# mic-rud/RABBIT-Transcoding

Measured on AMD Instinct MI355X. Metric: transcoded point-cloud frames/sec, R5->R3, higher is better.
Workload: dtype u16/i32

## Files before the change

### rabbit-transcoding_amd/csrc/rbt_encode.h

```cpp
#pragma once
#include "rbt_cabac.h"
#include "rbt_recon.h"
#include "rbt_filter.h"

RBT_CONST uint16_t k_lambda16[76] = {3,    3,    4,    4,    5,    5,    6,    7,    8,    9,    10,   11,   12,   14,   15,   17,   19,   22,   24,
                                     27,   30,   34,   38,   43,   48,   54,   61,   68,   77,   86,   97,   108,  122,  137,  153,  172,  193,  217,
                                     244,  273,  307,  344,  387,  434,  487,  547,  614,  689,  773,  868,  974,  1093, 1227, 1378, 1546, 1736, 1948,
                                     2187, 2454, 2755, 3092, 3471, 3896, 4373, 4909, 5510, 6185, 6942, 7792, 8747, 9818, 11020, 12370, 13884, 15585, 17493};
RBT_CONST uint8_t k_intra_cand[11] = {0, 1, 26, 10, 2, 6, 14, 18, 22, 30, 34};
#define RBT_SPLIT_BITS 48
#define RBT_PARTIAL_COST 0x0FFFFFFF
#define RBT_AN_GOOD 2
#define RBT_AN_SKIPPED 0x0FFFFFFE

struct RbtEncLds {
  RbtReconLds rc;
  int16_t lvl[32 * 32];
};
struct RbtEntropyLds {
  uint8_t scan[3][4][64];
  uint8_t cu_l2[81], cu_md[81], cu_fl[81];
  alignas(16) int16_t lv[64 * 64 * 3 / 2];
};
#define RBT_ENTROPY_LDS_BYTES(tl2) (sizeof(RbtEntropyLds) - sizeof(int16_t) * (64 * 64 * 3 / 2 - (3 << (2 * (tl2) - 1))))
RBT_DEV RBT_LDS_AS int16_t* en_lv(RBT_LDS_AS RbtEntropyLds* l, int c, int log2_ctb) { const int nn = 1 << (2 * log2_ctb); return l->lv + (c == 0 ? 0 : c == 1 ? nn : nn + (nn >> 2)); }

RBT_DEV int en_wave_sum(int v, RBT_LDS_AS RbtEncLds* l) { (void)l; return rbt_wave_sum(v); }
#ifdef RBT_HOSTEMU
static inline int en_had8x8_sum_host(const int* r) {
  int t[64], sum = 0;
  for (int y = 0; y < 8; y++) for (int k = 0; k < 8; k++) { int s = 0; for (int x = 0; x < 8; x++) s += (__builtin_popcount(k & x) & 1) ? -r[y * 8 + x] : r[y * 8 + x]; t[y * 8 + k] = s; }
  for (int k = 0; k < 8; k++) for (int x = 0; x < 8; x++) { int s = 0; for (int y = 0; y < 8; y++) s += (__builtin_popcount(k & y) & 1) ? -t[y * 8 + x] : t[y * 8 + x]; sum += s < 0 ? -s : s; }
  return sum;
}
#define EN_HAD8X8_ACC(vr, acc) (acc) += en_had8x8_sum_host(vr)
#else
RBT_DEV int en_had_stage(int v, int partner, int upper) { return upper ? partner - v : partner + v; }
RBT_DEV int en_had8x8_abs(int v) {
  const int lane = (int)threadIdx.x & 63;
  v = en_had_stage(v, __builtin_amdgcn_update_dpp(0, v, 0x141, 0xF, 0xF, false), lane & 4);
  v = en_had_stage(v, __builtin_amdgcn_update_dpp(0, v, 0xB1, 0xF, 0xF, false), lane & 1);
  v = en_had_stage(v, __builtin_amdgcn_update_dpp(0, v, 0x4E, 0xF, 0xF, false), lane & 2);
  v = en_had_stage(v, __builtin_amdgcn_update_dpp(0, v, 0x128, 0xF, 0xF, false), lane & 8);
  v = en_had_stage(v, __builtin_amdgcn_ds_swizzle(v, 0x401F), lane & 16);
  v = en_had_stage(v, __builtin_amdgcn_ds_bpermute((lane ^ 32) << 2, v), lane & 32);
  return v < 0 ? -v : v;
}
#define EN_HAD8X8_ACC(vr, acc) (acc) += en_had8x8_abs(vr)
#endif
RBT_DEV int en_occ_unit(const RbtFrame* f, int ux, int uy) { return ux < f->occ4_w && uy < f->occ4_h && f->occ4[(size_t)uy * f->occ4_w + ux] != 0; }
RBT_DEV int en_round_mean(int sum, int cnt) { return sum >= 0 ? (sum + cnt / 2) / cnt : -((-sum + cnt / 2) / cnt); }
RBT_DEV int en_occ_unit_value(const uint16_t* occ, int ow, int oh, int s, int w4, int h4, int i, int j) {
  const int x_lo = (4 * rbt_max(i - 1, 0)) / s, x_hi = rbt_min(ow - 1, (4 * rbt_min(i + 1, w4 - 1) + 3) / s), y_lo = (4 * rbt_max(j - 1, 0)) / s, y_hi = rbt_min(oh - 1, (4 * rbt_min(j + 1, h4 - 1) + 3) / s);
  int any = 0;
  for (int y = y_lo; y <= y_hi; y++) for (int x = x_lo; x <= x_hi; x++) any |= occ[(size_t)y * ow + x] != 0;
  return any;
}
RBT_DEV int en_rq_offset(int lf_is0, int lf_is1, int xy_sum) { return lf_is0 ? (xy_sum <= 2 ? 180 : 145) : (lf_is1 ? 195 : 230); }
RBT_DEV int en_chroma_qp(const RbtFrame* f, const RbtSlice* sl, int c_idx, int qp_y) {
  int off = c_idx == 1 ? f->cfg.cb_qp_offset + sl->cb_qp_offset : f->cfg.cr_qp_offset + sl->cr_qp_offset;
  int bdo = 6 * (f->cfg.bit_depth - 8);
  int qpi = rbt_clip3(-bdo, 57, qp_y + off);
  return (qpi < 0 ? qpi : rbt_chroma_qp(qpi)) + bdo;
}

struct EnCtbNb { int cx, cy, ctb, w, h, left, above_left, above, above_right; };
RBT_DEV int en_avail(const EnCtbNb* q, int xc, int yc, int xn, int yn) {
  if (xn < 0 || yn < 0 || xn >= q->w || yn >= q->h) return 0;
  const int dx = xn - q->cx, dy = yn - q->cy;
  if (dy >= q->ctb) return 0;
  if (dy < 0) return dx < 0 ? q->above_left : (dx < q->ctb ? q->above : q->above_right);
  if (dx < 0) return q->left;
  if (dx >= q->ctb) return 0;
  return rc_z_before(dx >> 2, dy >> 2, (xc - q->cx) >> 2, (yc - q->cy) >> 2);
}
struct RbtAnalyseLds {
  int32_t nb[132], nbf[132], ref[100];
  uint16_t src[65 * 66];
  int32_t cost[3][16]; uint8_t mode[3][16], split[3][16];
  uint8_t hint[64];
};
RBT_DEV int en_nb_unit_av(const EnCtbNb* q, int p, int x0, int y0, int S) { int xn, yn; rc_nb_unit_xy(p, x0, y0, S, 0, &xn, &yn); return en_avail(q, x0, y0, xn, yn); }
RBT_DEV void en_analyse_ctb(RbtFrame* f, const RbtSlice* slices, int ctb_addr, RBT_LDS_AS RbtAnalyseLds* l) {
  const RbtStreamCfg gcopy = rc_cfg_uni(&f->cfg); const RbtStreamCfg* g = &gcopy;
  int ctb = 1 << g->log2_ctb, rx = ctb_addr % g->w_ctb, ry = ctb_addr / g->w_ctb, cx = rx << g->log2_ctb, cy = ry << g->log2_ctb;
  const int my_slice = f->ctb_slice[ctb_addr];
  const RbtSlice* sl = &slices[my_slice];
  RBT_LDS_AS RbtAnalyseLds* rl = l;
  EnCtbNb nbq; nbq.cx = cx; nbq.cy = cy; nbq.ctb = ctb; nbq.w = g->w; nbq.h = g->h;
  nbq.left = rx > 0 && f->ctb_slice[ctb_addr - 1] == my_slice;
  nbq.above = ry > 0 && f->ctb_slice[ctb_addr - g->w_ctb] == my_slice;
  nbq.above_left = rx > 0 && ry > 0 && f->ctb_slice[ctb_addr - g->w_ctb - 1] == my_slice;
  nbq.above_right = ry > 0 && rx + 1 < g->w_ctb && f->ctb_slice[ctb_addr - g->w_ctb + 1] == my_slice;
  const uint16_t* srcp = f->src[0];
  const int hints = f->hint_dm != nullptr, hint_w4 = f->hint_w4, hint_h4 = f->hint_h4, satd_on = f->enc_tools & RBT_ET_SATD;
  int nq = ctb > 32 ? 2 : 1, qs = ctb > 32 ? 32 : ctb;
  for (int q = 0; q < nq * nq; q++) {
    int qx = cx + (q % nq) * 32, qy = cy + (q / nq) * 32;
    if (nq > 1 && (qx >= g->w || qy >= g->h)) continue;
    if (!(RBT_ABLATE & 0x100))
#pragma unroll 4
    RBT_PAR_FOR(i, 65 * 16) {
      const int x4 = i & 15, yy = (i >> 4) - 1, x = qx + 4 * x4, y = qy + yy;
      RbtU2 v; v.x = 0; v.y = 0;
      if (y >= 0 && y < g->h && x < g->w) v = *(const RbtU2*)(srcp + (size_t)y * g->w + x);
      RBT_LDS_AS uint16_t* d = &l->src[(yy + 1) * 66 + 4 * x4 + 1];
      d[0] = (uint16_t)v.x; d[1] = (uint16_t)(v.x >> 16); d[2] = (uint16_t)v.y; d[3] = (uint16_t)(v.y >> 16);
    }
    RBT_PAR_FOR(i, 65) { const int x = qx - 1, y = qy + i - 1; l->src[i * 66] = (x >= 0 && y >= 0 && y < g->h) ? srcp[(size_t)y * g->w + x] : 0; }
    if (hints && !(RBT_ABLATE & 0x400)) RBT_PAR_FOR(u, 64) {
      const int hx = (qx >> 2) + (u & 7), hy = (qy >> 2) + (u >> 3); int v = 255;
      if (hx < hint_w4 && hy < hint_h4) { const size_t hk = (size_t)hy * hint_w4 + hx; if ((f->hint_pm[hk] & RBT_PM_MODE_MASK) == RBT_MODE_INTRA) v = f->hint_dm[hk] & 63; }
      l->hint[u] = (uint8_t)v;
    }
    RBT_SYNC_LDS();
    for (int si = 2; si >= 0; si--) {
      int S = 8 << si; if (S > qs) continue;
      int nb = qs / S, lg = 3 + si;
      for (int b = 0; b < nb * nb; b++) {
        int x0 = qx + (b % nb) * S, y0 = qy + (b / nb) * S, best = 0x7FFFFFFF, bmode = 0;
        if (x0 >= g->w || y0 >= g->h) best = 0;
        else if (x0 + S > g->w || y0 + S > g->h) best = RBT_PARTIAL_COST;
        else if (si < 2 && 2 * S <= qs && (RBT_UNI(l->cost[si + 1][((b / nb) >> 1) * (nb >> 1) + ((b % nb) >> 1)]) <= (f->lossless ? 0 : RBT_AN_GOOD) * 4 * S * S ||
                                            RBT_UNI(l->cost[si + 1][((b / nb) >> 1) * (nb >> 1) + ((b % nb) >> 1)]) == RBT_AN_SKIPPED)) best = RBT_AN_SKIPPED;
        else {
          const int tot = 4 * S + 1, bx0 = x0 - qx, by0 = y0 - qy;
          if (!(RBT_ABLATE & 0x200)) {
          uint64_t m; RBT_VBALLOT(m, p, rc_nb_units(S, 0), en_nb_unit_av(&nbq, p, x0, y0, S));
          RcNbMap nm; rc_nb_map(&nm, m, S, 0);
          RBT_PAR_FOR(i, tot) {
            int v = 1 << (g->bit_depth - 1);
            if (m) { const int j = rc_nb_source(&nm, i); v = j < 2 * S ? l->src[(by0 + 2 * S - j) * 66 + bx0] : l->src[by0 * 66 + bx0 + j - 2 * S]; }
            rl->nb[i] = v;
          }
          RBT_SYNC_LDS();
          rc_intra_filter_apply(g, lg, rl->nb, rl->nbf);
          }
          int parent = -1;
          if (si == 0 && qs >= 16) { const int pb = ((b / nb) >> 1) * (nb >> 1) + ((b % nb) >> 1); if (RBT_UNI(l->cost[1][pb]) < RBT_PARTIAL_COST) parent = RBT_UNI(l->mode[1][pb]); }
          uint64_t hc = 0; int nh = 0;
          if (hints) {
            int any = 0;
            hc = 1ull << 6; nh = 2;
            if (!(RBT_ABLATE & 0x400)) for (int q = 0; q < 4; q++) {
              const int v = RBT_UNI(l->hint[((by0 + (q >> 1) * (S >> 1)) >> 2) * 8 + ((bx0 + (q & 1) * (S >> 1)) >> 2)]);
              if (v < 35) {
                any = 1;
                int dup = 0; for (int t = 0; t < nh; t++) dup |= (int)((hc >> (6 * t)) & 63) == v;
                if (!dup) { hc |= (uint64_t)v << (6 * nh); nh++; }
              }
            }
            if (!any) { hc |= (26ull << 12) | (10ull << 18); nh = 4; }
          }
          int coarse = 0;
          RBT_VEC(int, v_last); RBT_VEC(int, v_keep);
          RBT_VFOR(p, 64) { RBT_V(v_last, p) = 0; RBT_V(v_keep, p) = 0; }
          for (int k = 0; k < 15; k++) {
            int mode;
            if (best == 0) break;
            if (hints) { if (k >= nh) break; mode = (int)((hc >> (6 * k)) & 63); }
            else if (parent >= 0) {
              if (k >= 9) break;
              if (k < 4) mode = k == 0 ? 0 : (k == 1 ? 1 : (k == 2 ? 26 : 10));
              else if (parent >= 2) { mode = parent + (k - 6); if (mode < 2 || mode > 34 || mode == 10 || mode == 26) continue; }
              else { if (k >= 7) break; mode = k == 4 ? 2 : (k == 5 ? 18 : 34); }
            } else if (k < 11) mode = k_intra_cand[k];
            else { if (k == 11) coarse = bmode; if (coarse < 2) break; mode = coarse + (k == 11 ? -2 : k == 12 ? -1 : k == 13 ? 1 : 2); if (mode < 2 || mode > 34) continue; }
            RBT_LDS_AS int32_t* fin = rc_intra_filter_needed(0, lg, mode) ? rl->nbf : rl->nb;
            RcIntraCtx qc; if (!(RBT_ABLATE & 0x800)) rc_intra_setup(g, 0, lg, mode, fin, rl->ref, &qc); else { qc.N = S; qc.log2 = lg; qc.mode = mode; qc.c_idx = 0; qc.maxv = 1023; qc.ang = 1; qc.ver = mode >= 18; qc.dc = 1; qc.edge = 0; }
            int part = (RBT_ABLATE & 0x1000) ? 1 + k : 0;
#define EN_BODY(PV) RBT_PAR_FOR(i, S * S) { const int x = i & (S - 1), y = i >> lg, r = (int)l->src[(by0 + y + 1) * 66 + bx0 + x + 1] - (PV); part += rbt_abs(r); RBT_V(v_last, i & 63) = r; }
            if (!(RBT_ABLATE & 0x1000)) RC_INTRA_KINDS(&qc, fin, rl->ref, EN_BODY);
#undef EN_BODY
            int sad = en_wave_sum(part, (RBT_LDS_AS RbtEncLds*)0);
            if (sad < best) { best = sad; bmode = mode; if (S == 8) { RBT_VFOR(p, 64) RBT_V(v_keep, p) = RBT_V(v_last, p); } }
            RBT_SYNC_LDS();
          }
          if (satd_on && best > 0 && S == 8 && !(RBT_ABLATE & (0x2000 | 0x1000))) {
            int acc = 0; EN_HAD8X8_ACC(v_keep, acc);
            best = (en_wave_sum(acc, (RBT_LDS_AS RbtEncLds*)0) + 4) >> 3;
          } else if (satd_on && best > 0 && !(RBT_ABLATE & 0x2000)) {
            RBT_LDS_AS int32_t* fin = rc_intra_filter_needed(0, lg, bmode) ? rl->nbf : rl->nb;
            RcIntraCtx qc; rc_intra_setup(g, 0, lg, bmode, fin, rl->ref, &qc);
            int acc = 0; const int tw = S >> 3;
#define EN_BODY(PV) for (int tix = 0; tix < tw * tw; tix++) { \
              const int tx = (tix % tw) * 8, ty = (tix / tw) * 8; \
              RBT_VEC(int, v_r); \
              RBT_VFOR(p, 64) { const int x = tx + (p & 7), y = ty + (p >> 3); RBT_V(v_r, p) = (int)l->src[(by0 + y + 1) * 66 + bx0 + x + 1] - (PV); } \
              EN_HAD8X8_ACC(v_r, acc); }
            RC_INTRA_KINDS(&qc, fin, rl->ref, EN_BODY);
#undef EN_BODY
            best = (en_wave_sum(acc, (RBT_LDS_AS RbtEncLds*)0) + 4) >> 3;
            RBT_SYNC_LDS();
          }
        }
    if (RBT_LANE0) { l->cost[si][b] = best; l->mode[si][b] = (uint8_t)bmode; }
      }
    }
    RBT_SYNC_LDS();
    int lam = k_lambda16[rbt_clip3(0, 75, sl->qp + 6 * (g->bit_depth - 8))], pen = (lam * RBT_SPLIT_BITS) >> 4;
    for (int si = 1; si < 3; si++) {
      int S = 8 << si; if (S > qs) break;
      int nb = qs / S, nbc = nb * 2;
      RBT_PAR_FOR(b, nb * nb) {
        int bx = b % nb, by = b / nb;
        int child = l->cost[si - 1][(2 * by) * nbc + 2 * bx] + l->cost[si - 1][(2 * by) * nbc + 2 * bx + 1] + l->cost[si - 1][(2 * by + 1) * nbc + 2 * bx] +
                    l->cost[si - 1][(2 * by + 1) * nbc + 2 * bx + 1] + pen;
        int split = child < l->cost[si][b];
        l->split[si][b] = (uint8_t)split;
        if (split) l->cost[si][b] = child;
      }
      RBT_SYNC_LDS();
    }
    int n8 = qs / 8;
    RBT_PAR_FOR(u, n8 * n8) {
      int ux = u % n8, uy = u / n8, x = qx + ux * 8, y = qy + uy * 8;
      if (x < g->w && y < g->h) {
        int lg = 3, mode = l->mode[0][uy * n8 + ux];
        int inside32 = qx + 32 <= g->w && qy + 32 <= g->h, inside16 = (x & ~15) + 16 <= g->w && (y & ~15) + 16 <= g->h;
        int b16 = (uy / 2) * (n8 / 2) + ux / 2;
        int split32 = qs >= 32 ? (inside32 ? l->split[2][0] : 1) : 1;
        int split16 = qs >= 16 ? (inside16 ? l->split[1][b16] : 1) : 1;
        if (qs >= 32 && !split32) { lg = 5; mode = l->mode[2][0]; }
        else if (qs >= 16 && !split16) { lg = 4; mode = l->mode[1][b16]; }
        int k = (y >> 3) * f->w8 + (x >> 3);
        f->cu_log2[k] = (uint8_t)lg; f->cu_mode[k] = (uint8_t)mode;
      }
    }
    RBT_SYNC_LDS();
  }
}

template <int LOG2> RBT_DEV void en_fwd_transform_n(int is_dst, int bd, RBT_LDS_AS RbtReconLdsCore* r) {
  constexpr int N = 1 << LOG2; const int s1 = LOG2 + bd - 9, s2 = LOG2 + 6;
  RBT_PAR_FOR(i, N * N) {
    int k = i & (N - 1), y = i >> LOG2, s = 0;
#pragma unroll
    for (int x = 0; x < N; x++) s += rc_tcoef(r, N, is_dst, k, x) * r->res[y * N + x];
    r->tmp[i] = (int16_t)(s1 > 0 ? (s + (1 << (s1 - 1))) >> s1 : s);
  }
  RBT_SYNC_LDS();
  RBT_PAR_FOR(i, N * N) {
    int kh = i & (N - 1), kv = i >> LOG2, s = 0;
#pragma unroll
    for (int y = 0; y < N; y++) s += rc_tcoef(r, N, is_dst, kv, y) * r->tmp[y * N + kh];
    r->res[i] = (int16_t)rbt_clip3(-32768, 32767, (s + (1 << (s2 - 1))) >> s2);
  }
  RBT_SYNC_LDS();
}
template <int LOG2> RBT_DEV void en_fwd_transform_pair_n(int bd, RBT_LDS_AS RbtReconLdsCore* r) {
  constexpr int N = 1 << LOG2, NN = N * N; const int s1 = LOG2 + bd - 9, s2 = LOG2 + 6;
  RBT_PAR_FOR(i, 2 * NN) {
    const int b = i >> (2 * LOG2), j = i & (NN - 1), k = j & (N - 1), y = j >> LOG2; int s = 0;
#pragma unroll
    for (int x = 0; x < N; x++) s += rc_tcoef(r, N, 0, k, x) * r->res[b * 256 + y * N + x];
    r->tmp[b * 256 + j] = (int16_t)(s1 > 0 ? (s + (1 << (s1 - 1))) >> s1 : s);
  }
  RBT_SYNC_LDS();
  RBT_PAR_FOR(i, 2 * NN) {
    const int b = i >> (2 * LOG2), j = i & (NN - 1), kh = j & (N - 1), kv = j >> LOG2; int s = 0;
#pragma unroll
    for (int y = 0; y < N; y++) s += rc_tcoef(r, N, 0, kv, y) * r->tmp[b * 256 + y * N + kh];
    r->res[b * 256 + j] = (int16_t)rbt_clip3(-32768, 32767, (s + (1 << (s2 - 1))) >> s2);
  }
  RBT_SYNC_LDS();
}
RBT_DEV void en_fwd_transform_32(int bd, RBT_LDS_AS RbtReconLdsCore* r) {
#ifdef RBT_HOSTEMU
  en_fwd_transform_n<5>(0, bd, r);
#else
  mf_mm32<false>(r->dct, 32, 1, r->res, r->tmp, 5 + bd - 9, 0);
  mf_mm32<true>(r->dct, 32, 1, r->tmp, r->res, 5 + 6, 1);
#endif
}
RBT_DEV void en_fwd_transform(int log2, int is_dst, int bd, RBT_LDS_AS RbtReconLdsCore* r) {
  if (log2 == 2) en_fwd_transform_n<2>(is_dst, bd, r);
  else if (log2 == 3) en_fwd_transform_n<3>(0, bd, r);
  else if (log2 == 4) en_fwd_transform_n<4>(0, bd, r);
  else en_fwd_transform_32(bd, r);
}
RBT_DEV int en_quant(int log2, int qp, int bd, int is_intra, RBT_LDS_AS RbtEncLds* l) {
  int N = 1 << log2, qbits = 14 + qp / 6 + (15 - bd - log2), sc = k_quant_scale[qp % 6], part = 0;
  long long add = (long long)(is_intra ? 171 : 85) << (qbits - 9);
  RBT_PAR_FOR(i, N * N) {
    int c = l->rc.res[i], a = rbt_abs(c);
    long long q = ((long long)a * sc + add) >> qbits;
    if (q > 32767) q = 32767;
    l->lvl[i] = (int16_t)(c < 0 ? -q : q);
    part += q != 0;
  }
  int nz = en_wave_sum(part, l);
  return nz;
}
RBT_DEV int en_code_tb(RbtFrame* f, int c_idx, int x0, int y0, int log2, int qp, int is_intra, RBT_LDS_AS RbtEncLds* l) {
  const RbtStreamCfg* g = &f->cfg;
  int N = 1 << log2, pw = c_idx ? g->cw : g->w, bd = g->bit_depth, maxv = (1 << bd) - 1;
  const uint16_t* sp = f->src[c_idx]; uint16_t* rp = f->pix[c_idx]; int16_t* cp = f->coef[c_idx];
  RBT_PAR_FOR(i, N * N) { int x = i & (N - 1), y = i >> log2; l->rc.res[i] = (int16_t)((int)sp[(size_t)(y0 + y) * pw + x0 + x] - (int)l->rc.pred[i]); }
  RBT_SYNC_LDS();
  int occ_none = 0;
  if (f->occ4 != nullptr) {
    const int sh = c_idx ? 1 : 0;
#define EN_TBP_OCC(i) en_occ_unit(f, ((x0 + ((i) & (N - 1))) << sh) >> 2, ((y0 + ((i) >> log2)) << sh) >> 2)
    int pc = 0, ps = 0;
    RBT_PAR_FOR(i, N * N) { if (EN_TBP_OCC(i)) { pc++; ps += l->rc.res[i]; } }
    const int cnt = en_wave_sum(pc, l);
    occ_none = cnt == 0;
    if (cnt > 0 && cnt < N * N) {
      const int mean = en_round_mean(en_wave_sum(ps, l), cnt);
      RBT_PAR_FOR(i, N * N) { if (!EN_TBP_OCC(i)) l->rc.res[i] = (int16_t)mean; }
      RBT_SYNC_LDS();
    }
#undef EN_TBP_OCC
  }
  int nz;
  if (occ_none) { RBT_PAR_FOR(i, N * N) l->lvl[i] = 0; nz = 0; }
  else if (f->lossless) {
    int part = 0;
    RBT_PAR_FOR(i, N * N) { l->lvl[i] = l->rc.res[i]; part += l->rc.res[i] != 0; }
    nz = en_wave_sum(part, l);
  } else {
    en_fwd_transform(log2, c_idx == 0 && log2 == 2 && is_intra, bd, &l->rc);
    nz = en_quant(log2, qp, bd, is_intra, l);
  }
  RBT_SYNC_LDS();
  if (nz) { RBT_PAR_FOR(i, N * N) { int x = i & (N - 1), y = i >> log2; cp[(size_t)(y0 + y) * pw + x0 + x] = l->lvl[i]; } }
  if (nz && !f->lossless) {
    int bd_shift = bd + log2 - 5, scale = (16 * k_dequant_scale[qp % 6]) << (qp / 6);
    long long add = 1ll << (bd_shift - 1);
    RBT_PAR_FOR(i, N * N) { long long v = ((long long)l->lvl[i] * scale + add) >> bd_shift; l->rc.res[i] = (int16_t)(v < -32768 ? -32768 : (v > 32767 ? 32767 : v)); }
// ... 1066 lines not shown
```

### rabbit-transcoding_amd/csrc/rbt_recon.h

```cpp
#pragma once
#include "rbt_tables.h"
#include "rbt_types.h"
#include "rbt_mfma.h"

struct RbtReconLdsCore {
  int32_t nb[132];
  alignas(16) int16_t res[32 * 32];
  alignas(16) int16_t tmp[32 * 32];
  int8_t dct[32 * 32]; int8_t dst[16];
};
struct RbtReconLds : RbtReconLdsCore {
  int32_t nbf[132];
  int32_t ref[100];
  int32_t ref2[100];
  uint16_t pred[32 * 32];
};
RBT_DEV void rc_stage_tables(RBT_LDS_AS RbtReconLdsCore* l) {
  RBT_PAR_FOR(i, 1024) l->dct[i] = k_dct32[i >> 5][i & 31];
  RBT_PAR_FOR(i, 16) l->dst[i] = k_dst4[i >> 2][i & 3];
  RBT_SYNC_LDS();
}

RBT_DEV int rc_morton(int x4, int y4) {
  int z = 0;
  for (int b = 0; b < 4; b++) z |= (((x4 >> b) & 1) << (2 * b)) | (((y4 >> b) & 1) << (2 * b + 1));
  return z;
}
RBT_DEV int rc_z_before(int ax, int ay, int bx, int by) {
  const int dx = ax ^ bx, dy = ay ^ by, x_decides = dy < dx && dy < (dx ^ dy);
  return x_decides ? ax < bx : ay < by;
}
RBT_DEV int rc_avail(const RbtFrame* f, int xc, int yc, int xn, int yn) {
  const RbtStreamCfg* g = &f->cfg;
  if (xn < 0 || yn < 0 || xn >= g->w || yn >= g->h) return 0;
  int L = g->log2_ctb, an = (yn >> L) * g->w_ctb + (xn >> L), ac = (yc >> L) * g->w_ctb + (xc >> L);
  if (an > ac || f->ctb_slice[an] != f->ctb_slice[ac]) return 0;
  if (an == ac) {
    int m = (1 << L) - 1;
    if (rc_morton((xn & m) >> 2, (yn & m) >> 2) >= rc_morton((xc & m) >> 2, (yc & m) >> 2)) return 0;
  }
  if (g->cip && (f->pm[(yn >> 2) * g->w4 + (xn >> 2)] & RBT_PM_MODE_MASK) != RBT_MODE_INTRA) return 0;
  return 1;
}
RBT_DEV int rc_tcoef(const RBT_LDS_AS RbtReconLdsCore* l, int N, int is_dst, int k, int n) { return is_dst ? l->dst[k * 4 + n] : l->dct[k * (32 / N) * 32 + n]; }

RBT_DEV int rc_intra_angle(int mode) {
  const int k = mode <= 18 ? mode - 2 : 34 - mode, d = k < 8 ? 8 - k : k - 8;
  const uint64_t M = 0ull | (2ull << 6) | (5ull << 12) | (9ull << 18) | (13ull << 24) | (17ull << 30) | (21ull << 36) | (26ull << 42) | (32ull << 48);
  const int a = (int)((M >> (6 * d)) & 63);
  return k <= 8 ? a : -a;
}
RBT_DEV int rc_intra_inv_angle(int mode) {
  const int d = mode < 18 ? 18 - mode : mode - 18;
  const uint64_t lo = 256ull | (315ull << 16) | (390ull << 32) | (482ull << 48), hi = 630ull | (910ull << 16) | (1638ull << 32) | (4096ull << 48);
  return -(int)(((d < 4 ? lo : hi) >> (16 * (d & 3))) & 0xFFFF);
}
RBT_DEV int rc_level_scale(int r) { return (int)((0x484039332D28ull >> (8 * r)) & 255); }
RBT_DEV int rbt_wave_sum(int v) {
#ifdef RBT_HOSTEMU
  return v;
#else
  int x = v;
  x += __builtin_amdgcn_update_dpp(0, x, 0xB1, 0xF, 0xF, false);
  x += __builtin_amdgcn_update_dpp(0, x, 0x4E, 0xF, 0xF, false);
  x += __builtin_amdgcn_update_dpp(0, x, 0x141, 0xF, 0xF, false);
  x += __builtin_amdgcn_update_dpp(0, x, 0x140, 0xF, 0xF, false);
  return __builtin_amdgcn_readlane(x, 0) + __builtin_amdgcn_readlane(x, 16) + __builtin_amdgcn_readlane(x, 32) + __builtin_amdgcn_readlane(x, 48);
#endif
}
struct RcNbMap { uint64_t m; int two_n, usl, nu, lo, hi, run; };
RBT_DEV int rc_nb_unit_of(const RcNbMap* q, int i) { return i < q->two_n ? i >> q->usl : (i == q->two_n ? q->nu : q->nu + 1 + ((i - q->two_n - 1) >> q->usl)); }
RBT_DEV int rc_nb_unit_lo(const RcNbMap* q, int u) { return u < q->nu ? u << q->usl : (u == q->nu ? q->two_n : q->two_n + 1 + ((u - q->nu - 1) << q->usl)); }
RBT_DEV int rc_nb_unit_hi(const RcNbMap* q, int u) { return u < q->nu ? (u << q->usl) + (1 << q->usl) - 1 : (u == q->nu ? q->two_n : q->two_n + ((u - q->nu) << q->usl)); }
RBT_DEV void rc_nb_unit_xy(int p, int x0, int y0, int N, int sh, int* xn, int* yn) {
  const int usl = 2 - sh, nu = (2 * N) >> usl;
  if (p < nu) { *xn = x0 - 1; *yn = y0 + 2 * N - 1 - (p << usl); }
  else if (p == nu) { *xn = x0 - 1; *yn = y0 - 1; }
  else { *xn = x0 + ((p - nu - 1) << usl); *yn = y0 - 1; }
}
RBT_DEV int rc_nb_units(int N, int sh) { return ((4 * N) >> (2 - sh)) + 1; }
RBT_DEV void rc_nb_map(RcNbMap* q, uint64_t m, int N, int sh) {
  q->m = m; q->two_n = 2 * N; q->usl = 2 - sh; q->nu = (2 * N) >> q->usl; q->lo = q->hi = -1; q->run = 0;
  if (m) {
    const int ua = __builtin_ctzll(m), ub = 63 - __builtin_clzll(m); const uint64_t t = m >> ua;
    q->lo = rc_nb_unit_lo(q, ua); q->hi = rc_nb_unit_hi(q, ub); q->run = (t & (t + 1)) == 0;
  }
}
RBT_DEV int rc_nb_source(const RcNbMap* q, int i) {
  if (q->run) return rbt_clip3(q->lo, q->hi, i);
  const int u = rc_nb_unit_of(q, i); const uint64_t t = q->m & ((2ull << u) - 1);
  if (!t) return q->lo;
  const int uj = 63 - __builtin_clzll(t);
  return uj == u ? i : rc_nb_unit_hi(q, uj);
}
RBT_DEV int rc_intra_filter_needed(int c_idx, int log2, int mode) {
  const int N = 1 << log2;
  if (c_idx != 0 || mode == 1 || N == 4) return 0;
  const int md = rbt_min(rbt_abs(mode - 26), rbt_abs(mode - 10)), thr = N == 8 ? 7 : (N == 16 ? 1 : 0);
  return md > thr;
}
RBT_DEV void rc_intra_filter_apply(const RbtStreamCfg* g, int log2, RBT_LDS_AS int32_t* nb, RBT_LDS_AS int32_t* alt) {
  const int N = 1 << log2, bd = g->bit_depth, tot = 4 * N + 1;
  int corner = nb[2 * N], bl = nb[0], tr = nb[4 * N];
  int strong = g->strong_intra && N == 32 && rbt_abs(corner + tr - 2 * nb[2 * N + 32]) < (1 << (bd - 5)) &&
               rbt_abs(corner + bl - 2 * nb[2 * N - 32]) < (1 << (bd - 5));
  RBT_PAR_FOR(i, tot) {
    int v;
    if (i == 0 || i == 4 * N) v = nb[i];
    else if (strong) {
      if (i == 2 * N) v = corner;
      else if (i < 2 * N) { int k = 2 * N - 1 - i; v = ((63 - k) * corner + (k + 1) * bl + 32) >> 6; }
      else { int k = i - 2 * N - 1; v = ((63 - k) * corner + (k + 1) * tr + 32) >> 6; }
    } else v = (nb[i - 1] + 2 * nb[i] + nb[i + 1] + 2) >> 2;
    alt[i] = v;
  }
  RBT_SYNC_LDS();
}
RBT_DEV RBT_LDS_AS int32_t* rc_intra_filter(const RbtStreamCfg* g, int c_idx, int log2, int mode, RBT_LDS_AS int32_t* nb, RBT_LDS_AS int32_t* alt) {
  if (!rc_intra_filter_needed(c_idx, log2, mode)) return nb;
  if (!(RBT_ABLATE & 4)) rc_intra_filter_apply(g, log2, nb, alt);
  return alt;
}
struct RcIntraCtx { int N, log2, mode, c_idx, maxv, ang, ver, dc, edge; };
RBT_DEV void rc_intra_setup(const RbtStreamCfg* g, int c_idx, int log2, int mode, RBT_LDS_AS int32_t* nb, RBT_LDS_AS int32_t* ref, RcIntraCtx* q) {
  const int N = 1 << log2, bd = g->bit_depth;
  q->N = N; q->log2 = log2; q->mode = mode; q->c_idx = c_idx; q->maxv = (1 << bd) - 1; q->ang = 0; q->ver = mode >= 18; q->dc = 0; q->edge = 0;
#define RC_LEFT(y) nb[2 * N - 1 - (y)]
#define RC_TOP(x) nb[2 * N + 1 + (x)]
  if (mode == 1) {
    int part = 0;
    if (!(RBT_ABLATE & 8)) RBT_PAR_FOR(p, 2 * N) part += p < N ? RC_TOP(p) : RC_LEFT(p - N);
    q->dc = (N + rbt_wave_sum(part)) >> (log2 + 1); q->edge = c_idx == 0 && N < 32;
  } else if (mode >= 2) {
    const int ang = rc_intra_angle(mode), ver = mode >= 18, last = (N * ang) >> 5;
    const int inv = (mode >= 11 && mode <= 25) ? rc_intra_inv_angle(mode) : 0;
    q->ang = ang; q->edge = c_idx == 0 && N < 32 && (mode == 26 || mode == 10);
    if (!(RBT_ABLATE & 8)) RBT_PAR_FOR(i, 3 * N + 1) {
      int x = i - N, v = 0;
      if (x >= 0 && x <= N) v = ver ? RC_TOP(x - 1) : RC_LEFT(x - 1);
      else if (x < 0) { if (ang < 0 && last < -1 && x >= last) { int k = -1 + ((x * inv + 128) >> 8); v = ver ? RC_LEFT(k) : RC_TOP(k); } }
      else if (ang >= 0) v = ver ? RC_TOP(x - 1) : RC_LEFT(x - 1);
      ref[x + 32] = v;
    }
    RBT_SYNC_LDS();
  }
}
RBT_DEV int rc_pred_planar(const RcIntraCtx* q, const RBT_LDS_AS int32_t* nb, int x, int y) {
  const int N = q->N;
  return ((N - 1 - x) * RC_LEFT(y) + (x + 1) * RC_TOP(N) + (N - 1 - y) * RC_TOP(x) + (y + 1) * RC_LEFT(N) + N) >> (q->log2 + 1);
}
RBT_DEV int rc_pred_dc_edge(const RcIntraCtx* q, const RBT_LDS_AS int32_t* nb, int x, int y) {
  const int N = q->N; int v = q->dc;
  if (x == 0 && y == 0) v = (RC_LEFT(0) + 2 * q->dc + RC_TOP(0) + 2) >> 2;
  else if (y == 0) v = (RC_TOP(x) + 3 * q->dc + 2) >> 2;
  else if (x == 0) v = (RC_LEFT(y) + 3 * q->dc + 2) >> 2;
  return v;
}
template <int VER> RBT_DEV int rc_pred_angular(const RcIntraCtx* q, const RBT_LDS_AS int32_t* ref, int x, int y) {
  const int a = VER ? y : x, b = VER ? x : y, t = (a + 1) * q->ang, idx = t >> 5, fr = t & 31;
  return ((32 - fr) * ref[32 + b + idx + 1] + fr * ref[32 + b + idx + 2] + 16) >> 5;
}
RBT_DEV int rc_pred_angular_edge(const RcIntraCtx* q, const RBT_LDS_AS int32_t* nb, const RBT_LDS_AS int32_t* ref, int x, int y) {
  const int N = q->N; int v = ref[32 + (q->ver ? x : y) + 1];
  if (q->mode == 26 && x == 0) v = rbt_clip3(0, q->maxv, RC_TOP(0) + ((RC_LEFT(y) - RC_LEFT(-1)) >> 1));
  if (q->mode == 10 && y == 0) v = rbt_clip3(0, q->maxv, RC_LEFT(0) + ((RC_TOP(x) - RC_TOP(-1)) >> 1));
  return v;
}
#define RC_INTRA_KINDS(q, nb, ref, BODY) do { \
    if ((q)->mode == 0) { BODY(rc_pred_planar((q), (nb), x, y)) } \
    else if ((q)->mode == 1) { if ((q)->edge) { BODY(rc_pred_dc_edge((q), (nb), x, y)) } else { BODY((q)->dc) } } \
    else if ((q)->edge) { BODY(rc_pred_angular_edge((q), (nb), (ref), x, y)) } \
    else if ((q)->ver) { BODY(rc_pred_angular<1>((q), (ref), x, y)) } \
    else { BODY(rc_pred_angular<0>((q), (ref), x, y)) } } while (0)
#define RC_INTRA_KINDS_PAIR(qu, ql, nb, ref, BODY) do { \
    if ((qu)->mode == 0) { BODY(rc_pred_planar((ql), (nb), x, y)) } \
    else if ((qu)->mode == 1) { BODY((ql)->dc) } \
    else if ((qu)->ver) { BODY(rc_pred_angular<1>((ql), (ref), x, y)) } \
    else { BODY(rc_pred_angular<0>((ql), (ref), x, y)) } } while (0)
#undef RC_LEFT
#undef RC_TOP
template <class CP> RBT_DEV void rc_dequant(CP plane, int pst, int x0, int y0, int log2, int qp, int bd, RBT_LDS_AS RbtReconLdsCore* l) {
  int N = 1 << log2, bd_shift = bd + log2 - 5;
  int scale = (16 * rc_level_scale(qp % 6)) << (qp / 6);
  long long add = 1ll << (bd_shift - 1);
  RBT_PAR_FOR(i, N * N) {
    int x = i & (N - 1), y = i >> log2;
    long long v = ((long long)plane[(size_t)(y0 + y) * pst + x0 + x] * scale + add) >> bd_shift;
    l->res[i] = (int16_t)(v < -32768 ? -32768 : (v > 32767 ? 32767 : v));
  }
  RBT_SYNC_LDS();
}
template <int LOG2> RBT_DEV void rc_inv_transform_n(int is_dst, int sh, RBT_LDS_AS RbtReconLdsCore* l) {
  constexpr int N = 1 << LOG2;
  RBT_PAR_FOR(i, N * N) {
    int x = i & (N - 1), y = i >> LOG2, s = 0;
#pragma unroll
    for (int k = 0; k < N; k++) s += rc_tcoef(l, N, is_dst, k, y) * l->res[k * N + x];
    l->tmp[i] = (int16_t)rbt_clip3(-32768, 32767, (s + 64) >> 7);
  }
  RBT_SYNC_LDS();
  RBT_PAR_FOR(i, N * N) {
    int x = i & (N - 1), y = i >> LOG2, s = 0;
#pragma unroll
    for (int k = 0; k < N; k++) s += rc_tcoef(l, N, is_dst, k, x) * l->tmp[y * N + k];
    l->res[i] = (int16_t)rbt_clip3(-32768, 32767, (s + (1 << (sh - 1))) >> sh);
  }
  RBT_SYNC_LDS();
}
RBT_DEV void rc_inv_transform_32(int sh, RBT_LDS_AS RbtReconLdsCore* l) {
#ifdef RBT_HOSTEMU
  rc_inv_transform_n<5>(0, sh, l);
#else
  mf_mm32<true>(l->dct, 1, 32, l->res, l->tmp, 7, 1);
  mf_mm32<false>(l->dct, 1, 32, l->tmp, l->res, sh, 1);
#endif
}
RBT_DEV void rc_inv_transform(int log2, int is_dst, int ts, int bd, RBT_LDS_AS RbtReconLdsCore* l) {
  int N = 1 << log2, sh = 20 - bd;
  if (ts) {
    RBT_PAR_FOR(i, N * N) l->res[i] = (int16_t)(((int)l->res[i] * 128 + (1 << (sh - 1))) >> sh);
    RBT_SYNC_LDS();
    return;
  }
  if (log2 == 2) rc_inv_transform_n<2>(is_dst, sh, l);
  else if (log2 == 3) rc_inv_transform_n<3>(0, sh, l);
  else if (log2 == 4) rc_inv_transform_n<4>(0, sh, l);
  else rc_inv_transform_32(sh, l);
}

template <int LOG2> RBT_DEV void rc_inv_transform_pair_n(int sh, int m0, int m1, RBT_LDS_AS RbtReconLdsCore* l) {
  constexpr int N = 1 << LOG2, NN = N * N;
  RBT_PAR_FOR(i, 2 * NN) {
    const int b = i >> (2 * LOG2), j = i & (NN - 1), x = j & (N - 1), y = j >> LOG2;
    if (b ? m1 : m0) {
// ... 370 lines not shown
```

Measured before the change: 1025.

## Precompute interior-CTB neighbour runs and batch 8x8 hinted intra SAD evaluation

For interior CTBs, reference-sample availability is read from a compile-time constexpr table instead of a per-block ballot and neighbour map. Hinted 8x8 blocks now evaluate all candidate modes in one pass, packing residuals as 16-bit values in registers. The SADs are reduced together with a batched DPP/swizzle multi-value wave sum, replacing a per-mode LDS-synchronised loop. This trades higher register pressure and added code complexity for fewer barriers and reductions in the analysis kernel.

```diff
diff --git a/rabbit-transcoding_amd/csrc/rbt_encode.h b/rabbit-transcoding_amd/csrc/rbt_encode.h
--- a/rabbit-transcoding_amd/csrc/rbt_encode.h
+++ b/rabbit-transcoding_amd/csrc/rbt_encode.h
@@ -65,7 +65,7 @@
 }
 
 struct EnCtbNb { int cx, cy, ctb, w, h, left, above_left, above, above_right; };
-RBT_DEV int en_avail(const EnCtbNb* q, int xc, int yc, int xn, int yn) {
+RBT_DEV constexpr int en_avail(const EnCtbNb* q, int xc, int yc, int xn, int yn) {
   if (xn < 0 || yn < 0 || xn >= q->w || yn >= q->h) return 0;
   const int dx = xn - q->cx, dy = yn - q->cy;
   if (dy >= q->ctb) return 0;
@@ -80,7 +80,79 @@
   int32_t cost[3][16]; uint8_t mode[3][16], split[3][16];
   uint8_t hint[64];
 };
-RBT_DEV int en_nb_unit_av(const EnCtbNb* q, int p, int x0, int y0, int S) { int xn, yn; rc_nb_unit_xy(p, x0, y0, S, 0, &xn, &yn); return en_avail(q, x0, y0, xn, yn); }
+static_assert(sizeof(RbtAnalyseLds) <= 10388, "RbtAnalyseLds must not grow: 14 workgroups per CU is the analysis kernel's design point");
+RBT_DEV constexpr int en_nb_unit_av(const EnCtbNb* q, int p, int x0, int y0, int S) { int xn = 0, yn = 0; rc_nb_unit_xy(p, x0, y0, S, 0, &xn, &yn); return en_avail(q, x0, y0, xn, yn); }
+#define EN_AN_NB_NO_RUN 0xFFFFFFFFu
+RBT_DEV constexpr int en_an_nb_index(int log2_ctb, int q, int si, int b) { return (log2_ctb - 4 + q) * 21 + (si == 0 ? 0 : (si == 1 ? 16 : 20)) + b; }
+RBT_DEV constexpr uint32_t en_an_nb_entry(int log2_ctb, int q, int si, int b) {
+  const int ctb = 1 << log2_ctb, nq = ctb > 32 ? 2 : 1, qs = ctb > 32 ? 32 : ctb, S = 8 << si;
+  if (S > qs || b >= (qs / S) * (qs / S) || q >= nq * nq) return 0;
+  EnCtbNb n{}; n.cx = n.cy = 4 * ctb; n.ctb = ctb; n.w = n.h = 16 * ctb; n.left = n.above_left = n.above = n.above_right = 1;
+  const int x0 = n.cx + (q % nq) * 32 + (b % (qs / S)) * S, y0 = n.cy + (q / nq) * 32 + (b / (qs / S)) * S;
+  uint64_t m = 0;
+  for (int p = 0; p < rc_nb_units(S, 0); p++) if (en_nb_unit_av(&n, p, x0, y0, S)) m |= 1ull << p;
+  RcNbMap nm{}; rc_nb_map(&nm, m, S, 0);
+  return nm.run ? (uint32_t)nm.lo | (uint32_t)nm.hi << 8 : EN_AN_NB_NO_RUN;
+}
+struct EnAnNbTable { uint32_t e[6 * 21]; };
+RBT_DEV constexpr EnAnNbTable en_an_nb_table() {
+  EnAnNbTable t{};
+  for (int lc = 4; lc <= 6; lc++) for (int q = 0; q < (lc == 6 ? 4 : 1); q++) for (int si = 0; si < 3; si++) for (int b = 0; b < (si == 0 ? 16 : (si == 1 ? 4 : 1)); b++)
+    t.e[en_an_nb_index(lc, q, si, b)] = en_an_nb_entry(lc, q, si, b);
+  return t;
+}
+RBT_DEV constexpr int en_an_nb_all_runs(const EnAnNbTable& t) { for (int i = 0; i < 6 * 21; i++) if (t.e[i] == EN_AN_NB_NO_RUN) return 0; return 1; }
+RBT_CONST EnAnNbTable k_an_nb = en_an_nb_table();
+static_assert(en_an_nb_all_runs(en_an_nb_table()), "the available reference units of a block of an interior CTB form one run");
+#ifdef RBT_HOSTEMU
+extern "C" { inline uint32_t rbt_hostemu_analysis[5]; }
+#define EN_AN_COUNT(k, on) do { if (on) __atomic_fetch_add(&rbt_hostemu_analysis[k], 1u, __ATOMIC_RELAXED); } while (0)
+extern "C" {
+__attribute__((used)) inline uint32_t rbt_hostemu_an_nb_entry(int log2_ctb, int q, int si, int b) { return k_an_nb.e[en_an_nb_index(log2_ctb, q, si, b)]; }
+__attribute__((used)) inline uint32_t rbt_hostemu_an_nb_ballot(int w, int h, int log2_ctb, int rx, int ry, int q, int si, int b) {
+  const int ctb = 1 << log2_ctb, w_ctb = (w + ctb - 1) >> log2_ctb, nq = ctb > 32 ? 2 : 1, qs = ctb > 32 ? 32 : ctb, S = 8 << si;
+  EnCtbNb n; n.cx = rx << log2_ctb; n.cy = ry << log2_ctb; n.ctb = ctb; n.w = w; n.h = h;
+  n.left = rx > 0; n.above = ry > 0; n.above_left = rx > 0 && ry > 0; n.above_right = ry > 0 && rx + 1 < w_ctb;
+  const int x0 = n.cx + (q % nq) * 32 + (b % (qs / S)) * S, y0 = n.cy + (q / nq) * 32 + (b / (qs / S)) * S;
+  uint64_t m; RBT_VBALLOT(m, p, rc_nb_units(S, 0), en_nb_unit_av(&n, p, x0, y0, S));
+  RcNbMap nm; rc_nb_map(&nm, m, S, 0);
+  return (uint32_t)(nm.lo & 255) | (uint32_t)(nm.hi & 255) << 8 | (uint32_t)nm.run << 16 | (uint32_t)(m != 0) << 17;
+}
+}
+#else
+#define EN_AN_COUNT(k, on) do { } while (0)
+#endif
+template <int NV> RBT_DEV void en_wave_sums(int (&v)[NV]) {
+#ifndef RBT_HOSTEMU
+  constexpr int H = NV / 2, Q = NV / 4;
+  const int lane = (int)threadIdx.x & 63, b0 = lane & 1, b1 = lane & 2;
+  int a[H], c[Q];
+#pragma unroll
+  for (int k = 0; k < H; k++) { const int keep = b0 ? v[k + H] : v[k], send = b0 ? v[k] : v[k + H]; a[k] = keep + __builtin_amdgcn_update_dpp(0, send, 0xB1, 0xF, 0xF, false); }
+#pragma unroll
+  for (int k = 0; k < Q; k++) { const int keep = b1 ? a[k + Q] : a[k], send = b1 ? a[k] : a[k + Q]; c[k] = keep + __builtin_amdgcn_update_dpp(0, send, 0x4E, 0xF, 0xF, false); }
+#pragma unroll
+  for (int k = 0; k < Q; k++) {
+    c[k] += __builtin_amdgcn_update_dpp(0, c[k], 0x124, 0xF, 0xF, false);
+    c[k] += __builtin_amdgcn_update_dpp(0, c[k], 0x128, 0xF, 0xF, false);
+    c[k] += __builtin_amdgcn_ds_swizzle(c[k], 0x401F);
+    c[k] += __builtin_amdgcn_ds_bpermute((lane ^ 32) << 2, c[k]);
+  }
+#pragma unroll
+  for (int j = 0; j < NV; j++) v[j] = __builtin_amdgcn_readlane(c[j % Q], (j / H) | (((j % H) / Q) << 1));
+#endif
+}
+template <int NEG> RBT_DEV int en_pred8_angular(const RBT_LDS_AS int32_t* fin, int ang, int inv, int ver, int x, int y) {
+  const int a = ver ? y : x, b = ver ? x : y, t = (a + 1) * ang, fr = t & 31, i0 = b + (t >> 5) + 1, i1 = rbt_min(i0 + 1, 16);
+  int e0 = i0, e1 = i1;
+  if (NEG) { if (i0 < 0) e0 = -((i0 * inv + 128) >> 8); if (i1 < 0) e1 = -((i1 * inv + 128) >> 8); }
+  if (!ver) { e0 = -e0; e1 = -e1; }
+  return ((32 - fr) * fin[16 + e0] + fr * fin[16 + e1] + 16) >> 5;
+}
+RBT_DEV int en_pred8_pure(const RBT_LDS_AS int32_t* nb, int ver, int maxv, int x, int y) {
+  if (ver) return x == 0 ? rbt_clip3(0, maxv, nb[17] + ((nb[15 - y] - nb[16]) >> 1)) : nb[17 + x];
+  return y == 0 ? rbt_clip3(0, maxv, nb[15] + ((nb[17 + x] - nb[16]) >> 1)) : nb[15 - y];
+}
 RBT_DEV void en_analyse_ctb(RbtFrame* f, const RbtSlice* slices, int ctb_addr, RBT_LDS_AS RbtAnalyseLds* l) {
   const RbtStreamCfg gcopy = rc_cfg_uni(&f->cfg); const RbtStreamCfg* g = &gcopy;
   int ctb = 1 << g->log2_ctb, rx = ctb_addr % g->w_ctb, ry = ctb_addr / g->w_ctb, cx = rx << g->log2_ctb, cy = ry << g->log2_ctb;
@@ -92,6 +164,7 @@
   nbq.above = ry > 0 && f->ctb_slice[ctb_addr - g->w_ctb] == my_slice;
   nbq.above_left = rx > 0 && ry > 0 && f->ctb_slice[ctb_addr - g->w_ctb - 1] == my_slice;
   nbq.above_right = ry > 0 && rx + 1 < g->w_ctb && f->ctb_slice[ctb_addr - g->w_ctb + 1] == my_slice;
+  const int interior = RBT_UNI(g->log2_ctb >= 4 && nbq.left && nbq.above_left && nbq.above && nbq.above_right && cx + 2 * ctb <= g->w && cy + ctb <= g->h);
   const uint16_t* srcp = f->src[0];
   const int hints = f->hint_dm != nullptr, hint_w4 = f->hint_w4, hint_h4 = f->hint_h4, satd_on = f->enc_tools & RBT_ET_SATD;
   int nq = ctb > 32 ? 2 : 1, qs = ctb > 32 ? 32 : ctb;
@@ -126,12 +199,18 @@
         else {
           const int tot = 4 * S + 1, bx0 = x0 - qx, by0 = y0 - qy;
           if (!(RBT_ABLATE & 0x200)) {
+          EN_AN_COUNT(interior ? 0 : 1, 1);
+          if (interior) {
+            const uint32_t e = k_an_nb.e[en_an_nb_index(g->log2_ctb, q, si, b)]; const int lo = (int)(e & 255), hi = (int)(e >> 8);
+            RBT_PAR_FOR(i, tot) { const int j = rbt_clip3(lo, hi, i); rl->nb[i] = j < 2 * S ? l->src[(by0 + 2 * S - j) * 66 + bx0] : l->src[by0 * 66 + bx0 + j - 2 * S]; }
+          } else {
           uint64_t m; RBT_VBALLOT(m, p, rc_nb_units(S, 0), en_nb_unit_av(&nbq, p, x0, y0, S));
           RcNbMap nm; rc_nb_map(&nm, m, S, 0);
           RBT_PAR_FOR(i, tot) {
             int v = 1 << (g->bit_depth - 1);
             if (m) { const int j = rc_nb_source(&nm, i); v = j < 2 * S ? l->src[(by0 + 2 * S - j) * 66 + bx0] : l->src[by0 * 66 + bx0 + j - 2 * S]; }
             rl->nb[i] = v;
+          }
           }
           RBT_SYNC_LDS();
           rc_intra_filter_apply(g, lg, rl->nb, rl->nbf);
@@ -155,6 +234,47 @@
           int coarse = 0;
           RBT_VEC(int, v_last); RBT_VEC(int, v_keep);
           RBT_VFOR(p, 64) { RBT_V(v_last, p) = 0; RBT_V(v_keep, p) = 0; }
+          EN_AN_COUNT(2, nh == 6);
+#ifdef RBT_HOSTEMU
+          int n_min = 0;
+#define EN_AN_SEEN(sad) do { if ((sad) < best) n_min = 1; else if ((sad) == best) n_min++; } while (0)
+#else
+#define EN_AN_SEEN(sad) do { } while (0)
+#endif
+          if (hints && S == 8 && g->bit_depth <= 15 && !(RBT_ABLATE & (0x800 | 0x1000 | 0x2000))) {
+            int dsum = 0;
+            RBT_PAR_FOR(p, 16) dsum += rl->nb[p < 8 ? 17 + p : 23 - p];
+            RcIntraCtx qc; qc.N = 8; qc.log2 = 3; qc.mode = 0; qc.c_idx = 0; qc.maxv = (1 << g->bit_depth) - 1; qc.ang = 0; qc.ver = 0; qc.dc = (8 + rbt_wave_sum(dsum)) >> 4; qc.edge = 1;
+            RBT_VEC(int, v_src); RBT_VEC(uint32_t, v_p0); RBT_VEC(uint32_t, v_p1); RBT_VEC(uint32_t, v_p2);
+            RBT_VFOR(p, 64) { RBT_V(v_src, p) = (int)l->src[(by0 + (p >> 3) + 1) * 66 + bx0 + (p & 7) + 1]; RBT_V(v_p0, p) = 0; RBT_V(v_p1, p) = 0; RBT_V(v_p2, p) = 0; }
+#define EN_BODY8(PV) RBT_VFOR(p, 64) { const int x = p & 7, y = p >> 3, r = RBT_V(v_src, p) - (PV); \
+              RBT_V(v_p2, p) = RBT_V(v_p2, p) << 16 | RBT_V(v_p1, p) >> 16; RBT_V(v_p1, p) = RBT_V(v_p1, p) << 16 | RBT_V(v_p0, p) >> 16; RBT_V(v_p0, p) = RBT_V(v_p0, p) << 16 | ((uint32_t)r & 0xFFFFu); }
+            for (int k = 0; k < nh; k++) {
+              const int mode = (int)((hc >> (6 * k)) & 63);
+              const RBT_LDS_AS int32_t* fin = rc_intra_filter_needed(0, 3, mode) ? rl->nbf : rl->nb;
+              if (mode == 0) { EN_BODY8(rc_pred_planar(&qc, fin, x, y)) }
+              else if (mode == 1) { EN_BODY8(rc_pred_dc_edge(&qc, fin, x, y)) }
+              else if (mode == 10 || mode == 26) { EN_BODY8(en_pred8_pure(fin, mode == 26, qc.maxv, x, y)) }
+              else {
+                const int ang = rc_intra_angle(mode), ver = mode >= 18;
+                EN_AN_COUNT(4, ang < 0);
+                if (ang >= 0) { EN_BODY8(en_pred8_angular<0>(fin, ang, 0, ver, x, y)) }
+                else { const int inv = rc_intra_inv_angle(mode); EN_BODY8(en_pred8_angular<1>(fin, ang, inv, ver, x, y)) }
+              }
+            }
+#undef EN_BODY8
+            int sads[8] = {0, 0, 0, 0, 0, 0, 0, 0};
+            RBT_VFOR(p, 64) {
+              sads[0] += rbt_abs((int)(RBT_V(v_p0, p) << 16) >> 16); sads[1] += rbt_abs((int)RBT_V(v_p0, p) >> 16); sads[2] += rbt_abs((int)(RBT_V(v_p1, p) << 16) >> 16);
+              sads[3] += rbt_abs((int)RBT_V(v_p1, p) >> 16); sads[4] += rbt_abs((int)(RBT_V(v_p2, p) << 16) >> 16); sads[5] += rbt_abs((int)RBT_V(v_p2, p) >> 16);
+            }
+            if (nh <= 4) { int t4[4] = {sads[0], sads[1], sads[2], sads[3]}; en_wave_sums<4>(t4); sads[0] = t4[0]; sads[1] = t4[1]; sads[2] = t4[2]; sads[3] = t4[3]; }
+            else en_wave_sums<8>(sads);
+            int wf = 0;
+#pragma unroll
+            for (int fi = 5; fi >= 0; fi--) if (fi < nh) { EN_AN_SEEN(sads[fi]); if (sads[fi] < best) { best = sads[fi]; bmode = (int)((hc >> (6 * (nh - 1 - fi))) & 63); wf = fi; } }
+            RBT_VFOR(p, 64) { const uint32_t w = wf < 2 ? RBT_V(v_p0, p) : (wf < 4 ? RBT_V(v_p1, p) : RBT_V(v_p2, p)); RBT_V(v_keep, p) = (wf & 1) ? (int)w >> 16 : (int)(w << 16) >> 16; }
+          } else
           for (int k = 0; k < 15; k++) {
             int mode;
             if (best == 0) break;
@@ -173,9 +293,14 @@
             if (!(RBT_ABLATE & 0x1000)) RC_INTRA_KINDS(&qc, fin, rl->ref, EN_BODY);
 #undef EN_BODY
             int sad = en_wave_sum(part, (RBT_LDS_AS RbtEncLds*)0);
+            EN_AN_SEEN(sad);
             if (sad < best) { best = sad; bmode = mode; if (S == 8) { RBT_VFOR(p, 64) RBT_V(v_keep, p) = RBT_V(v_last, p); } }
             RBT_SYNC_LDS();
           }
+#undef EN_AN_SEEN
+#ifdef RBT_HOSTEMU
+          EN_AN_COUNT(3, best > 0 && n_min >= 2);
+#endif
           if (satd_on && best > 0 && S == 8 && !(RBT_ABLATE & (0x2000 | 0x1000))) {
             int acc = 0; EN_HAD8X8_ACC(v_keep, acc);
             best = (en_wave_sum(acc, (RBT_LDS_AS RbtEncLds*)0) + 4) >> 3;
diff --git a/rabbit-transcoding_amd/csrc/rbt_recon.h b/rabbit-transcoding_amd/csrc/rbt_recon.h
--- a/rabbit-transcoding_amd/csrc/rbt_recon.h
+++ b/rabbit-transcoding_amd/csrc/rbt_recon.h
@@ -26,7 +26,7 @@
   for (int b = 0; b < 4; b++) z |= (((x4 >> b) & 1) << (2 * b)) | (((y4 >> b) & 1) << (2 * b + 1));
   return z;
 }
-RBT_DEV int rc_z_before(int ax, int ay, int bx, int by) {
+RBT_DEV constexpr int rc_z_before(int ax, int ay, int bx, int by) {
   const int dx = ax ^ bx, dy = ay ^ by, x_decides = dy < dx && dy < (dx ^ dy);
   return x_decides ? ax < bx : ay < by;
 }
@@ -70,16 +70,16 @@
 }
 struct RcNbMap { uint64_t m; int two_n, usl, nu, lo, hi, run; };
 RBT_DEV int rc_nb_unit_of(const RcNbMap* q, int i) { return i < q->two_n ? i >> q->usl : (i == q->two_n ? q->nu : q->nu + 1 + ((i - q->two_n - 1) >> q->usl)); }
-RBT_DEV int rc_nb_unit_lo(const RcNbMap* q, int u) { return u < q->nu ? u << q->usl : (u == q->nu ? q->two_n : q->two_n + 1 + ((u - q->nu - 1) << q->usl)); }
-RBT_DEV int rc_nb_unit_hi(const RcNbMap* q, int u) { return u < q->nu ? (u << q->usl) + (1 << q->usl) - 1 : (u == q->nu ? q->two_n : q->two_n + ((u - q->nu) << q->usl)); }
-RBT_DEV void rc_nb_unit_xy(int p, int x0, int y0, int N, int sh, int* xn, int* yn) {
+RBT_DEV constexpr int rc_nb_unit_lo(const RcNbMap* q, int u) { return u < q->nu ? u << q->usl : (u == q->nu ? q->two_n : q->two_n + 1 + ((u - q->nu - 1) << q->usl)); }
+RBT_DEV constexpr int rc_nb_unit_hi(const RcNbMap* q, int u) { return u < q->nu ? (u << q->usl) + (1 << q->usl) - 1 : (u == q->nu ? q->two_n : q->two_n + ((u - q->nu) << q->usl)); }
+RBT_DEV constexpr void rc_nb_unit_xy(int p, int x0, int y0, int N, int sh, int* xn, int* yn) {
   const int usl = 2 - sh, nu = (2 * N) >> usl;
   if (p < nu) { *xn = x0 - 1; *yn = y0 + 2 * N - 1 - (p << usl); }
   else if (p == nu) { *xn = x0 - 1; *yn = y0 - 1; }
   else { *xn = x0 + ((p - nu - 1) << usl); *yn = y0 - 1; }
 }
-RBT_DEV int rc_nb_units(int N, int sh) { return ((4 * N) >> (2 - sh)) + 1; }
-RBT_DEV void rc_nb_map(RcNbMap* q, uint64_t m, int N, int sh) {
+RBT_DEV constexpr int rc_nb_units(int N, int sh) { return ((4 * N) >> (2 - sh)) + 1; }
+RBT_DEV constexpr void rc_nb_map(RcNbMap* q, uint64_t m, int N, int sh) {
   q->m = m; q->two_n = 2 * N; q->usl = 2 - sh; q->nu = (2 * N) >> q->usl; q->lo = q->hi = -1; q->run = 0;
   if (m) {
     const int ua = __builtin_ctzll(m), ub = 63 - __builtin_clzll(m); const uint64_t t = m >> ua;
```

After: 1034, median of 4. Within noise of the previous version (+0.9%).
